# WhatAShot/Electrocardio-Panorama

Measured on AMD Instinct MI355X. Metric: ECG-samples/sec (train step), higher is better.
Workload: dtype f32 (conv products: fp32 operands split into fp16 hi+lo = 22-23 bits, block-scaled, 3 fp16 matrix products each, fp32 accumulate; fp32-class, not IEEE fp32)

## Files before the change

electrocardio_panorama_amd/_lib.py:

```python
import ctypes as C
import os

import torch

_HERE = os.path.dirname(os.path.abspath(__file__))
LIB_PATH = os.path.join(_HERE, "csrc", "libnefnet_hip.so")

NEF_OK = 0
_ERR = {-1: "NEF_E_SHAPE", -2: "NEF_E_NULL", -3: "NEF_E_WORKSPACE", -4: "NEF_E_UNSUPPORTED"}

p = C.c_void_p
i32 = C.c_int
i64 = C.c_int64
f32 = C.c_float
sz = C.c_size_t


class ConvArgs(C.Structure):
    _fields_ = [
        ("x", p), ("wp", p), ("y", p), ("bias", p), ("in_scale", p), ("res", p), ("gate", p), ("mask", p),
        ("x_bs", i64), ("x_gs", i64), ("y_bs", i64), ("y_gs", i64), ("sc_bs", i64), ("sc_gs", i64),
        ("res_bs", i64), ("res_gs", i64), ("gate_bs", i64), ("gate_gs", i64),
        ("B", i32), ("T", i32), ("G", i32), ("Cin_g", i32), ("Cout_g", i32), ("K", i32),
        ("relu", i32), ("gate_scale", f32), ("drop_scale", f32), ("drop_p", f32), ("rng_seed", C.c_uint64),
# ... 92 lines not shown
    "nef_pass_combine_bwd": (i32, [p, p, i32, i32, i32, p]),
    "nef_pass_combine_stats_ws_bytes": (sz, [i32, i32]),
    "nef_pass_combine_fwd_stats": (i32, [p, p, p, p, p, p, p, p, p, p, p, p, sz, i32, i32, i32, f32, f32, p, p]),
    "nef_upsample2_fwd": (i32, [p, p, i64, i32, p]),
    "nef_upsample2_bwd": (i32, [p, p, i64, i32, p]),
    "nef_bn_ws_bytes": (sz, [i32, i32]),
    "nef_bn_train_stats": (i32, [p, p, p, p, p, p, p, p, p, p, sz, i32, i32, i32, i32, f32, f32, p, p]),
    "nef_conv_stats_slots": (i32, [i32, i32]),
    "nef_bn_stats_from_slots": (i32, [p, i32, p, p, p, p, p, p, p, p, p, sz, i32, i32, i32, i32, f32, f32, p, p]),
    "nef_bn_eval_affine": (i32, [p, p, p, p, p, p, i32, f32, p]),
    "nef_fold_bn": (i32, [p, p, p, p, p, p, i32, i32, p]),
    "nef_affine_relu_fwd": (i32, [p, p, p, p, i32, i32, i32, i32, p]),
    "nef_bn_bwd_ws_bytes": (sz, [C.POINTER(BnBwdArgs)]),
    "nef_bn_relu_bwd": (i32, [C.POINTER(BnBwdArgs), p]),
    "nef_bn_bwd_args_bytes": (sz, []),
    "nef_outconv_fwd": (i32, [p, p, p, i32, p, p, p, i32, i32, i32, p]),
    "nef_outconv_bwd_weight": (i32, [p, p, p, p, p, i32, p, p, p, sz, i32, i32, i32, p]),
    "nef_outconv_bwd_data": (i32, [p, p, p, p, i32, i32, i32, p]),
    "nef_outconv_bwd_weight_ws_bytes": (sz, [i32]),
    "nef_loss_ws_bytes": (sz, []),
    "nef_loss_fwd": (i32, [p, p, p, p, p, p, sz, i64, f32, f32, f32, i32, i32, p]),
    "nef_loss_bwd": (i32, [p, p, p, p, p, p, p, p, i64, f32, f32, f32, i32, i32, p]),
    "nef_loss_noise_fwd": (i32, [p, p, p, p, p, p, p, sz, i64, f32, f32, f32, i32, i32, p]),
    "nef_loss_noise_bwd": (i32, [p, p, p, p, p, p, p, p, p, i64, f32, f32, f32, i32, i32, p]),
    "nef_sgd_momentum": (i32, [p, p, p, i64, f32, f32, f32, i32, p, p, p, p]),
    "nef_adam": (i32, [p, p, p, p, i64, f32, C.c_double, C.c_double, f32, f32, f32, p, p, p, p, p]),
    "nef_update": (i32, [C.POINTER(UpdateArgs), p]),
    "nef_update_args_bytes": (sz, []),
    "nef_update_ema": (i32, [C.POINTER(UpdateArgs), C.POINTER(EmaArgs), p]),
    "nef_ema_args_bytes": (sz, []),
# ... 62 lines not shown
```

electrocardio_panorama_amd/csrc/elementwise.hip:

```cpp
#include "nef_common.h"
#include "roi_unpool.h"

namespace {

__global__ void chscale_fwd_kernel(const float* __restrict__ x, const float* __restrict__ s, int64_t s_bs,
                                   float* __restrict__ y, int B, int C, int T) {
    const int64_t rows = (int64_t)B * C;
    const int wave = threadIdx.x >> 6, lane = threadIdx.x & 63;
    for (int64_t row = (int64_t)blockIdx.x * 4 + wave; row < rows; row += (int64_t)gridDim.x * 4) {
        const int b = (int)(row / C), c = (int)(row % C);
        const float f = s[(int64_t)b * s_bs + c];
        const float* xr = x + row * T;
        float* yr = y + row * T;
        for (int t = lane; t < T; t += 64) yr[t] = xr[t] * f;
    }
}

__global__ void chscale_bwd_kernel(const float* __restrict__ gy, const float* __restrict__ x,
                                   const float* __restrict__ s, int64_t s_bs, float* __restrict__ gx,
                                   float* __restrict__ gs, int B, int C, int T, int relu_x) {
    const int64_t rows = (int64_t)B * C;
    const int wave = threadIdx.x >> 6, lane = threadIdx.x & 63;
    for (int64_t row = (int64_t)blockIdx.x * 4 + wave; row < rows; row += (int64_t)gridDim.x * 4) {
        const int b = (int)(row / C), c = (int)(row % C);
// ... 584 lines not shown
        const float af = a[p * C + c], bf = b[p * C + c];
        const float* xr = x + row * L;
        float* yr = y + row * L;
        for (int t = lane; t < L; t += 64) yr[t] = fmaxf(fmaf(xr[t], af, bf), 0.f);
    }
}

__global__ void outconv_go_kernel(const float* __restrict__ gout, const float* __restrict__ out, float* __restrict__ go,
                                  int64_t n) {
    for (int64_t i = (int64_t)blockIdx.x * blockDim.x + threadIdx.x; i < n; i += (int64_t)gridDim.x * blockDim.x) {
        const float o = out[i];
        go[i] = gout[i] * (o * (1.f - o)) / 3.0f;
    }
}

__device__ __forceinline__ nef_f32x4 oc_grad4(const float* __restrict__ gor, int t4, int L, float w0, float w1, float w2) {
    const nef_f32x4 m = *(const nef_f32x4*)(gor + 4 * t4);
    const float lo = t4 > 0 ? gor[4 * t4 - 1] : 0.f;
    const float hi = 4 * t4 + 4 < L ? gor[4 * t4 + 4] : 0.f;
    nef_f32x4 g;
    g[0] = w0 * m[1] + w1 * m[0] + w2 * lo;
    g[1] = w0 * m[2] + w1 * m[1] + w2 * m[0];
    g[2] = w0 * m[3] + w1 * m[2] + w2 * m[1];
    g[3] = w0 * hi + w1 * m[3] + w2 * m[2];
    return g;
}

__device__ __forceinline__ nef_f32x4 up2_adjoint4(const float* __restrict__ gr, int t4, int L) {
    const nef_f32x4 v0 = *(const nef_f32x4*)(gr + 8 * t4), v1 = *(const nef_f32x4*)(gr + 8 * t4 + 4);
    const float lo = t4 > 0 ? gr[8 * t4 - 1] : 0.f;
    const float hi = 8 * t4 + 8 < 2 * L ? gr[8 * t4 + 8] : 0.f;
    nef_f32x4 g;
    g[0] = 0.25f * lo + 0.75f * v0[0] + 0.75f * v0[1] + 0.25f * v0[2];
    g[1] = 0.25f * v0[1] + 0.75f * v0[2] + 0.75f * v0[3] + 0.25f * v1[0];
    g[2] = 0.25f * v0[3] + 0.75f * v1[0] + 0.75f * v1[1] + 0.25f * v1[2];
    g[3] = 0.25f * v1[1] + 0.75f * v1[2] + 0.75f * v1[3] + 0.25f * hi;
    if (t4 == 0) g[0] = up2_bwd_edge(gr, L, 0);
    if (4 * t4 + 3 == L - 1) g[3] = up2_bwd_edge(gr, L, L - 1);
    return g;
}

template <int MODE>
__global__ __launch_bounds__(256) void bn_bwd_partial(const float* __restrict__ gy, const float* __restrict__ x,
                                                      const float* __restrict__ mean, const float* __restrict__ invstd,
                                                      const float* __restrict__ a, const float* __restrict__ b,
                                                      double* __restrict__ part, int P, int Bp, int C, int L,
                                                      const float* __restrict__ ocw) {
    __shared__ double sm[4];
    int bid = blockIdx.x;
    const int sp = bid % BN_SPLIT;
    bid /= BN_SPLIT;
    const int c = bid % C;
    const int p = bid / C;
    const float mf = mean[p * C + c], is = invstd[p * C + c], af = a[p * C + c], bf = b[p * C + c];
    constexpr bool OC = MODE == 1, UPG = MODE == 2;
    const float w0 = OC ? ocw[c * 3] : 0.f, w1 = OC ? ocw[c * 3 + 1] : 0.f, w2 = OC ? ocw[c * 3 + 2] : 0.f;
    double s1 = 0.0, s2 = 0.0;
    if ((L & 3) == 0) {
        const int L4 = L >> 2;
        for (int bb = sp; bb < Bp; bb += BN_SPLIT) {
            const int64_t off = (((int64_t)p * Bp + bb) * C + c) * L;
            const nef_f32x4* xr = (const nef_f32x4*)(x + off);
            const nef_f32x4* gr = (const nef_f32x4*)(gy + off);
            const float* gor = gy + ((int64_t)p * Bp + bb) * L;
            const float* gur = gy + 2 * off;
#pragma unroll 2
            for (int t = threadIdx.x; t < L4; t += 256) {
                const nef_f32x4 xv = xr[t],
                                gv = OC ? oc_grad4(gor, t, L, w0, w1, w2) : (UPG ? up2_adjoint4(gur, t, L) : gr[t]);
#pragma unroll
                for (int e = 0; e < 4; ++e) {
                    const float g = fmaf(xv[e], af, bf) > 0.f ? gv[e] : 0.f;
                    s1 += (double)g;
                    s2 += (double)g * (double)((xv[e] - mf) * is);
                }
            }
        }
    } else {
        for (int bb = sp; bb < Bp; bb += BN_SPLIT) {
            const int64_t off = (((int64_t)p * Bp + bb) * C + c) * L;
            for (int t = threadIdx.x; t < L; t += 256) {
                const float xv = x[off + t];
                const float g = fmaf(xv, af, bf) > 0.f ? gy[off + t] : 0.f;
                s1 += (double)g;
                s2 += (double)g * (double)((xv - mf) * is);
            }
        }
    }
    s1 = nef_block_sum_d(s1, sm);
    s2 = nef_block_sum_d(s2, sm);
    if (threadIdx.x == 0) {
        part[((int64_t)(p * C + c) * BN_SPLIT + sp) * 2] = s1;
        part[((int64_t)(p * C + c) * BN_SPLIT + sp) * 2 + 1] = s2;
    }
}

__global__ void bn_bwd_final(const double* __restrict__ part, float* __restrict__ coef, float* __restrict__ ggamma,
                             float* __restrict__ gbeta, int P, int Bp, int C, int L, int nsplit = BN_SPLIT) {
    const int c = blockIdx.x * blockDim.x + threadIdx.x;
    if (c >= C) return;
    const double n = (double)Bp * (double)L;
    double g1 = 0.0, g2 = 0.0;
    for (int p = 0; p < P; ++p) {
        double s1 = 0.0, s2 = 0.0;
        for (int sp = 0; sp < nsplit; ++sp) {
            s1 += part[((int64_t)(p * C + c) * nsplit + sp) * 2];
            s2 += part[((int64_t)(p * C + c) * nsplit + sp) * 2 + 1];
        }
        coef[(p * C + c) * 2] = (float)(s1 / n);
// ... 136 lines not shown
    double rs[3] = {0.0, 0.0, 0.0};
    for (int t = threadIdx.x; t < L; t += 256) {
        float o[3];
#pragma unroll
        for (int p = 0; p < 3; ++p) {
            const float xv = xr[p][t];
            const float g = fmaf(xv, af[p], bf[p]) > 0.f ? gr[p][t] : 0.f;
            o[p] = af[p] * (g - k1[p] - (xv - mf[p]) * is[p] * k2[p]);
            rs[p] += (double)o[p];
        }
        const int tq = deint ? (t & 1) * (L >> 1) + (t >> 1) : t;
        am[tq] = o[0] + o[2];
        ap[tq] = o[1];
        bm[tq] = o[0] + o[1];
        bp[tq] = o[2];
    }
    if (rowsum) {
#pragma unroll
        for (int p = 0; p < 3; ++p) {
            const double v = nef_block_sum_d(rs[p], sm);
            if (threadIdx.x == 0) rowsum[((int64_t)p * Bp + bb) * C + c] = v;
        }
    }
}

__global__ __launch_bounds__(256) void rowsum_to_channel(const double* __restrict__ rowsum, float* __restrict__ out,
                                                         int NB, int C) {
    __shared__ double sm[4];
    const int c = blockIdx.x;
    double s = 0.0;
// ... 1298 lines not shown
    NEF_REQUIRE(x && a && b && y, NEF_E_NULL);
    NEF_REQUIRE(P > 0 && Bp > 0 && C > 0 && L > 0, NEF_E_SHAPE);
    hipLaunchKernelGGL(affine_relu_fwd_kernel, dim3(nef_stream_grid((int64_t)P * Bp * C, 4)), dim3(256), 0, NEF_ST, x,
                       a, b, y, P, Bp, C, L);
    return nef_launch_status();
}

size_t nef_bn_bwd_args_bytes(void) { return sizeof(nef_bn_bwd_args); }

size_t nef_bn_bwd_ws_bytes(const nef_bn_bwd_args* a) {
    if (!a || a->form < 0 || a->form > 3 || a->P <= 0 || a->Bp <= 0 || a->C <= 0 || a->L <= 0) return 0;
    const size_t go = a->form == 1 ? (size_t)a->P * a->Bp * a->L * sizeof(float) : 0;
    return nef_bn_ws_bytes(a->P, a->C) + (size_t)a->P * a->Bp * a->C * sizeof(double) + go;
}

int nef_bn_relu_bwd(const nef_bn_bwd_args* args, nef_stream_t stream) {
    NEF_ENTER();
    NEF_REQUIRE(args, NEF_E_NULL);
    const nef_bn_bwd_args& a = *args;
    const int P = a.P, Bp = a.Bp, C = a.C, L = a.L, form = a.form, deint = a.phase_major;
    NEF_REQUIRE(a.x && a.mean && a.invstd && a.a && a.b && a.gx && a.ggamma && a.gbeta && a.ws, NEF_E_NULL);
    NEF_REQUIRE(form >= 0 && form <= 3, NEF_E_UNSUPPORTED);
    if (form == 1) {
        NEF_REQUIRE(a.gout && a.out && a.wout, NEF_E_NULL);
        NEF_REQUIRE(!a.g && !a.slots && !deint, NEF_E_UNSUPPORTED);
    } else {
        NEF_REQUIRE(a.g, NEF_E_NULL);
        NEF_REQUIRE(!a.gout && !a.out && !a.wout && !(form == 2 && deint), NEF_E_UNSUPPORTED);
    }
    NEF_REQUIRE(P > 0 && Bp > 0 && C > 0 && L > 0, NEF_E_SHAPE);
    NEF_REQUIRE(form != 3 || P == 3, NEF_E_UNSUPPORTED);
    const int64_t rows = (int64_t)P * Bp * C;
    const bool by_rows = (L & 3) == 0 && rows <= 0x7FFFFFFF;
    switch (form) {
    case 0: NEF_REQUIRE(!deint || by_rows, NEF_E_SHAPE); break;
    case 1: NEF_REQUIRE(by_rows, NEF_E_SHAPE); break;
    case 2: NEF_REQUIRE(by_rows && L >= 8, NEF_E_SHAPE); break;
    case 3: NEF_REQUIRE((int64_t)Bp * C <= 0x7FFFFFFF && (!deint || (L & 1) == 0), NEF_E_SHAPE); break;
    }
    NEF_REQUIRE(!a.slots || (a.nslot > 0 && (int64_t)Bp * a.nslot <= 0x7FFFFFFF), NEF_E_SHAPE);
    NEF_REQUIRE(a.ws_bytes >= nef_bn_bwd_ws_bytes(args), NEF_E_WORKSPACE);
    double* part = (double*)a.ws;
    float* coef = (float*)((char*)a.ws + (size_t)P * C * BN_SPLIT * 2 * sizeof(double));
    double* rowsum = a.gx_chan_sum ? (double*)((char*)a.ws + nef_bn_ws_bytes(P, C)) : nullptr;
    const float* g = a.g;
    if (form == 1) {
        float* go = (float*)((char*)a.ws + nef_bn_ws_bytes(P, C) + (size_t)rows * sizeof(double));
        const int64_t n = (int64_t)P * Bp * L;
        hipLaunchKernelGGL(outconv_go_kernel, dim3(nef_stream_grid(n, 256)), dim3(256), 0, NEF_ST, a.gout, a.out, go, n);
        g = go;
    }
    if (a.slots) {
        hipLaunchKernelGGL(bn_slots_bwd_fused, dim3((unsigned)C), dim3(BNF_THREADS), 0, NEF_ST, a.slots, coef, a.ggamma, a.gbeta, P, Bp, C,
                           L, Bp * a.nslot);
    } else {
        const dim3 grid(P * C * BN_SPLIT);
        if (form == 1)
            hipLaunchKernelGGL(bn_bwd_partial<1>, grid, dim3(256), 0, NEF_ST, g, a.x, a.mean, a.invstd, a.a, a.b, part, P, Bp, C, L,
                               a.wout);
        else if (form == 2)
            hipLaunchKernelGGL(bn_bwd_partial<2>, grid, dim3(256), 0, NEF_ST, g, a.x, a.mean, a.invstd, a.a, a.b, part, P, Bp, C, L,
                               (const float*)nullptr);
        else
            hipLaunchKernelGGL(bn_bwd_partial<0>, grid, dim3(256), 0, NEF_ST, g, a.x, a.mean, a.invstd, a.a, a.b, part, P, Bp, C, L,
                               (const float*)nullptr);
        hipLaunchKernelGGL(bn_bwd_final, dim3((C + 63) / 64), dim3(64), 0, NEF_ST, (const double*)part, coef, a.ggamma, a.gbeta, P, Bp, C,
                           L, BN_SPLIT);
    }
    const dim3 grid((unsigned)rows);
    if (form == 3)
        hipLaunchKernelGGL(bn_bwd_apply_combine3, dim3((unsigned)(Bp * C)), dim3(256), 0, NEF_ST, g, a.x, a.mean, a.invstd, a.a, a.b,
                           (const float*)coef, a.gx, rowsum, Bp, C, L, deint);
    else if (form == 2)
        hipLaunchKernelGGL(bn_bwd_apply_rows<2>, grid, dim3(256), 0, NEF_ST, g, a.x, a.mean, a.invstd, a.a, a.b, (const float*)coef, a.gx,
                           rowsum, Bp, C, L >> 2, (const float*)nullptr);
    else if (form == 1)
        hipLaunchKernelGGL(bn_bwd_apply_rows<1>, grid, dim3(256), 0, NEF_ST, g, a.x, a.mean, a.invstd, a.a, a.b, (const float*)coef, a.gx,
                           rowsum, Bp, C, L >> 2, a.wout);
    else if (by_rows)
        hipLaunchKernelGGL(bn_bwd_apply_rows<0>, grid, dim3(256), 0, NEF_ST, g, a.x, a.mean, a.invstd, a.a, a.b, (const float*)coef, a.gx,
                           rowsum, Bp, C, L >> 2, (const float*)nullptr, deint);
    else
        hipLaunchKernelGGL(bn_bwd_apply, dim3(nef_stream_grid(rows, 4)), dim3(256), 0, NEF_ST, g, a.x, a.mean, a.invstd, a.a, a.b,
                           (const float*)coef, a.gx, rowsum, P, Bp, C, L);
    if (a.gx_chan_sum)
        hipLaunchKernelGGL(rowsum_to_channel, dim3(C), dim3(256), 0, NEF_ST, (const double*)rowsum, a.gx_chan_sum, P * Bp, C);
    return nef_launch_status();
}

int nef_outconv_fwd(const float* x, const float* a, const float* b, int Bp, const float* w, const float* bias,
                    float* out, int N, int C, int L, nef_stream_t stream) {
    NEF_ENTER();
    NEF_REQUIRE(x && w && bias && out, NEF_E_NULL);
    NEF_REQUIRE((a == nullptr) == (b == nullptr), NEF_E_NULL);
    NEF_REQUIRE(N > 0 && C > 0 && C <= OC_MAXC && L > 0 && (!a || Bp > 0), NEF_E_SHAPE);
    if ((L & 3) == 0) {
        const int tiles = (L + 1023) / 1024;
        hipLaunchKernelGGL(outconv_fwd_kernel<true>, dim3((unsigned)((int64_t)N * tiles)), dim3(256), 0, NEF_ST, x, w, bias,
                           out, N, C, L, tiles, a, b, a ? Bp : 1);
        return nef_launch_status();
    }
    const int tiles = (L + 255) / 256;
    hipLaunchKernelGGL(outconv_fwd_kernel<false>, dim3((unsigned)((int64_t)N * tiles)), dim3(256), 0, NEF_ST, x, w, bias,
                       out, N, C, L, tiles, a, b, a ? Bp : 1);
// ... 272 lines not shown
```

electrocardio_panorama_amd/csrc/roi.hip:

```cpp
#include "nef_common.h"
#include "roi_unpool.h"

namespace {

using namespace nef_unpool;

__device__ __forceinline__ float grid_x(const int64_t* __restrict__ roi_b, int j, int s, int T) {
    const float sc = (float)(2.0 / (double)T);
    const float r0 = ((float)roi_b[2 * j] * 0.25f) * sc + (-1.0f);
    const float r1 = ((float)roi_b[2 * j + 1] * 0.25f) * sc + (-1.0f);
    const float step = (r1 - r0) / (float)(BINS - 1);
    return s < BINS / 2 ? r0 + step * (float)s : r1 - step * (float)(BINS - 1 - s);
}

__device__ __forceinline__ float col_weight(float gx) {
    const float ix = ((gx + 1.f) * 1.f - 1.f) * 0.5f;
    const float x0 = floorf(ix);
    const float we = ix - x0;
    const float ww = 1.f - we;
    float w = 0.f;
    if (x0 == 0.f) w += ww;
    if (x0 + 1.f == 0.f) w += we;
    return w;
}
// ... 235 lines not shown
    constexpr int ROW = NSEG * SEGW;
    if (choice_dev) c2 = choice_dev[1];
    const int64_t rows = (int64_t)B * 128;
    const int wave = __builtin_amdgcn_readfirstlane((int)(threadIdx.x >> 6)), lane = threadIdx.x & 63;
    const int s = lane & (SEGW - 1), half = lane >> 5;
    const int64_t per_wave = (rows + (int64_t)gridDim.x * 4 - 1) / ((int64_t)gridDim.x * 4);
    const int64_t row_lo = ((int64_t)blockIdx.x * 4 + wave) * per_wave;
    const int64_t row_hi = row_lo + per_wave < rows ? row_lo + per_wave : rows;
    float* sa = strip_lds + wave * (2 * T + ROW);
    float* sb = sa + T;
    float* pick = sb + T;
    const float fv = (float)V;
    const int64_t pass = (int64_t)B * 256 * T;
    int b_cur = -1;
    SegTable st;
    for (int64_t row = row_lo; row < row_hi; ++row) {
        const int b = (int)(row >> 7), c = (int)(row & 127);
        if (b != b_cur) {
            b_cur = b;
            load_segments(rois + (int64_t)b * NSEG * 2, T, st);
        }
        const float* zr = z2b + (((int64_t)b * V + c2) * 128 + c) * ROW;
#pragma unroll
        for (int u = 0; u < 4; ++u)
            if (u * 64 + lane < ROW) pick[u * 64 + lane] = zr[u * 64 + lane];
        __builtin_amdgcn_fence(__ATOMIC_RELEASE, "wavefront");
        __builtin_amdgcn_wave_barrier();
        const int64_t grow = ((int64_t)b * 256 + 128 + c) * T;
        const float f = q[b * 256 + 128 + c];
        float acc = 0.f;
        constexpr int NU = G == 4 ? 6 : (G == 2 ? 10 : 20);
        const int shift = G == 4 ? (c & 1) * T : 0;
        const int kb = shift / G, ke = (shift + T + G - 1) / G;
        for (int k0 = (kb & ~63) + lane; k0 < ke; k0 += 64 * NU) {
            float ga[NU][G], gb[NU][G], la[NU][G];
// ... 32 lines not shown
                        if (segment_of(st, t, i, sc, jb)) {
                            lerp_src(i, sc, i0, i1, l0, l1);
                            pk = unpool_lerp(l0, pick[jb + i0], l1, pick[jb + i1]);
                        }
                        acc += ga[u][e] * la[u][e] + gb[u][e] * pk;
                        const float gm = f * ga[u][e] / fv;
                        sa[t] = gm + 0.f;
                        sb[t] = gm + f * gb[u][e];
                    }
                }
            }
        }
        __builtin_amdgcn_fence(__ATOMIC_RELEASE, "wavefront");
        __builtin_amdgcn_wave_barrier();
        float ra[(NSEG + 1) / 2] = {0.f, 0.f, 0.f, 0.f}, rb[(NSEG + 1) / 2] = {0.f, 0.f, 0.f, 0.f};
        unpool_gather_row(sa, st, lane, ra);
        unpool_gather_row(sb, st, lane, rb);
        for (int v = 0; v < V; ++v) {
            float* gz = gz2b + (((int64_t)b * V + v) * 128 + c) * ROW;
#pragma unroll
            for (int k = 0; k < (NSEG + 1) / 2; ++k)
                if (2 * k + half < NSEG) gz[(2 * k + half) * SEGW + s] = v == c2 ? rb[k] : ra[k];
        }
        acc = nef_wave_sum(acc);
        if (lane == 0) gq[b * 256 + 128 + c] = acc;
        __builtin_amdgcn_wave_barrier();
    }
}

__global__ void roi_segment_table_kernel(const int64_t* __restrict__ rois, int64_t* __restrict__ seg_start,
                                         int64_t* __restrict__ seg_len, int n) {
    const int i = blockIdx.x * blockDim.x + threadIdx.x;
// ... 101 lines not shown
```

electrocardio_panorama_amd/csrc/roi_unpool.h:

```cpp
#pragma once
#include "nef_common.h"

namespace nef_unpool {

constexpr int NSEG = NEF_N_SEG;
constexpr int BINS = NEF_ROI_BINS;
constexpr int SEGW = 2 * NEF_ROI_BINS;

__device__ __forceinline__ int64_t latent_index(int64_t roi) {
    return (int64_t)((float)roi * 0.25f);
}

struct SegTable { int start[NSEG]; int len[NSEG]; int off[NSEG]; float scale[NSEG]; };

__device__ __forceinline__ bool load_segments(const int64_t* __restrict__ roi_b, int T, SegTable& st) {
    int run = 0;
    bool ok = true;
#pragma unroll
    for (int j = 0; j < NSEG; ++j) {
        const int64_t a = latent_index(roi_b[2 * j]);
        const int64_t e = latent_index(roi_b[2 * j + 1]);
        int64_t len = e - a;
        if (len < 0) { ok = false; len = 0; }
        if (run + len > T) { ok = false; len = T - run; }
// ... 31 lines not shown
    if (s <= 0) return 0;
    int i = (int)ceilf(((float)s + 0.5f) * inv_scale - 0.5f);
    if (i < 0) i = 0;
    if (i > len) i = len;
    if (i > 0 && unpool_left_tap(i - 1, scale) >= s) --i;
    else if (i < len && unpool_left_tap(i, scale) < s) ++i;
    if ((i > 0 && unpool_left_tap(i - 1, scale) >= s) || (i < len && unpool_left_tap(i, scale) < s)) {
#pragma nounroll
        while (i > 0 && unpool_left_tap(i - 1, scale) >= s) --i;
#pragma nounroll
        while (i < len && unpool_left_tap(i, scale) < s) ++i;
    }
    return i;
}

__device__ __forceinline__ void unpool_gather_row(const float* gr, const SegTable& st, int lane, float (&acc_out)[(NSEG + 1) / 2]) {
    const int s = lane & (SEGW - 1), half = lane >> 5;
#pragma unroll
    for (int jj = 0; jj < NSEG + 1; jj += 2) {
        const int j = jj + half;
        if (j >= NSEG) continue;
        const int len = half ? st.len[jj + 1 < NSEG ? jj + 1 : jj] : st.len[jj];
        const int off = half ? st.off[jj + 1 < NSEG ? jj + 1 : jj] : st.off[jj];
        const float sc = half ? st.scale[jj + 1 < NSEG ? jj + 1 : jj] : st.scale[jj];
        float acc = 0.f;
        if (len > 0) {
            const int b0 = unpool_first_reaching(s, len, sc, (float)len * (1.f / SEGW));
            const int nb = __shfl_down(b0, 1), pb = __shfl_up(b0, 1);
            const int b1 = s + 1 < SEGW ? nb : len;
            const int a0 = s > 0 ? pb : b0;
            const float* gp = gr + off;
            float fi = (float)a0 + 0.5f;
            const float sm1 = (float)(s - 1);
            for (int i = a0; i < b0; ++i, fi += 1.f) {
                float src = sc * fi - 0.5f;
                src = src < 0.f ? 0.f : src;
                acc += (src - sm1) * gp[i];
            }
            const float c0 = s == SEGW - 1 ? 1.f : (float)(s + 1), k = s == SEGW - 1 ? 0.f : 1.f;
            for (int i = b0; i < b1; ++i, fi += 1.f) {
                float src = sc * fi - 0.5f;
                src = src < 0.f ? 0.f : src;
                acc += (c0 - k * src) * gp[i];
            }
        }
        acc_out[jj >> 1] = acc;
    }
}

}

NEF_HIDDEN void nef_unpool_mix_fwd_z2(const float* z2b, const int64_t* rois, const float* q, float* latent, float* D2, int32_t* status,
                                      int B, int V, int T, int c2, const int32_t* choice_dev, hipStream_t st);
NEF_HIDDEN void nef_unpool_mix_bwd_z2(const float* gD, const float* latent, const float* z2b, const int64_t* rois, const float* q,
                                      float* gz2b, float* gq, int B, int V, int T, int c2, const int32_t* choice_dev, int group,
                                      hipStream_t st);
```

electrocardio_panorama_amd/engine.py:

```python
import os

import torch
from . import _env

from . import ops
from .ops import GV

N_SEG, ROI_BINS = 7, 16
DROP_P = 0.2
BN_EPS, BN_MOM = 1e-5, 0.1


DROPOUT_SITES = ("W_encoder.layer1.0", "W_encoder.layer1.1", "W_encoder.layer1.2", "w_conv.0", "z1_conv.0",
                 "z2_conv1.0", "z2_conv2.0", "z2_conv2.2")


class DropCfg:

    def __init__(self, training, p=DROP_P, masks=None, seed=0, seed_dev=None):
        self.seed_dev = seed_dev
        self.on = bool(training) and p > 0.0
        self.p = p if self.on else 0.0
        self.scale = 1.0 / (1.0 - p) if self.on else 1.0
        self.masks = masks
# ... 248 lines not shown
            mean = invstd = None
            Bp = N
        if save:
            saved.append((x_in, c, mean, invstd, a, b, pro, up_after, xedge))
        x, pro_in = c, (a, b, Bp)
    out = ops.outconv_fwd(x, P["decoder.4.weight"], P["decoder.4.bias"], pro=pro_in)
    return out, (saved, x, out, passes, pro_in, shared_B)


def decoder_bwd(dsaved, g_out, P, grads, side=None):
    saved, c4, out, passes, pro4 = dsaved[:5]
    shared_B = dsaved[5] if len(dsaved) > 5 else None
    side = side or ops._Inline()
    if len(dsaved) > 5:
        ops.pack_many(_decoder_pack_requests(P, c4.shape[2] // 4, True))
    grads["decoder.4.weight"], grads["decoder.4.bias"] = side.run(
        lambda: ops.outconv_bwd_weight(g_out, out, c4, pro=pro4), g_out, out, c4)
    fuse_last = c4.shape[2] % 4 == 0
    g_is_up = False
    g = None if fuse_last else ops.outconv_bwd_data(g_out, out, P["decoder.4.weight"], c4.shape[1])
    g_slots = None
    poly_first = False
    for li in (3, 2, 1, 0):
        blk, cv, bn, cout = _DEC[li]
        x, c, mean, invstd, a, b, pro, up_after = saved[li][:8]
        xedge = saved[li][8] if len(saved[li]) > 8 else None
        sh0 = li == 0 and shared_B is not None
        Cog_, Cig_ = c.shape[1], x.shape[1] // (2 if sh0 else 1)
        poly_b = bool(up_after and pro[0] & 2 and (not sh0 or pro[0] == 2) and ops.poly_bwd_ok(2 if sh0 else 1, Cog_, Cig_, c.shape[2]))
        pm = bool(poly_b and xedge is not None and ops.poly_w_ok((2 if sh0 else 1) * (shared_B if sh0 else c.shape[0]), 2 if sh0 else 1, Cog_, Cig_, c.shape[2]))
        wname, bname, pre = f"{blk}.double_conv.{cv}.weight", f"{blk}.double_conv.{cv}.bias", f"{blk}.double_conv.{bn}"
        pm0_done = False
        if li == 3 and fuse_last:
            gc, gg, gbeta, gbias = ops.bn_relu_bwd_outconv(g_out, out, P["decoder.4.weight"], c, mean, invstd, a, b, passes)
        elif li == 0 and shared_B is not None and not g_is_up:
            gc, gg, gbeta, gbias = ops.bn_relu_bwd_combine3(g, c, mean, invstd, a, b, slots=g_slots, phase_major=pm)
            pm0_done = pm
        elif g_is_up:
            gc, gg, gbeta, gbias = ops.bn_relu_bwd_up(g, c, mean, invstd, a, b, passes, slots=g_slots)
        else:
            gc, gg, gbeta, gbias = ops.bn_relu_bwd(g, c, P[pre + ".weight"], mean, invstd, a, b, passes,
                                                   with_chan_sum=True, slots=g_slots, phase_major=pm and not sh0)
            pm0_done = pm and not sh0
        grads[pre + ".weight"], grads[pre + ".bias"], grads[bname] = gg, gbeta, gbias
        pm = pm and pm0_done
        if li == 0 and shared_B is not None:
            gp2 = gc if gc.shape[0] == 2 * shared_B else ops.pass_combine_bwd(gc)
            gpv, xv = GV.dense(gp2, 2), GV.dense(x, 2)
            if pm:
# ... 363 lines not shown
```

electrocardio_panorama_amd/ops.py:

```python
import ctypes as C
import contextlib
import itertools
import os
from typing import NamedTuple, Optional

import torch
from . import _env

from . import _lib

N_SEG, ROI_BINS = 7, 16


def _p(t):
    return None if t is None else t.data_ptr()


def _stream():
    return torch.cuda.current_stream().cuda_stream


def _chk(t, dtype=torch.float32):
    assert t.is_cuda and t.dtype == dtype and t.is_contiguous(), (t.device, t.dtype, t.is_contiguous())
    return t
# ... 1249 lines not shown
    wf, bf = torch.empty_like(w), torch.empty_like(bias)
    _lib.check(L.nef_fold_bn(_p(w), _p(bias), _p(a), _p(b), _p(wf), _p(bf), w.shape[0], w.numel() // w.shape[0], _stream()),
               "nef_fold_bn")
    return wf, bf


def affine_relu_fwd(x, a, b, P):
    L = _lib.load()
    _chk(x)
    N, Ct, Ln = x.shape
    y = torch.empty_like(x)
    _lib.check(L.nef_affine_relu_fwd(_p(x), _p(a), _p(b), _p(y), P, N // P, Ct, Ln, _stream()), "nef_affine_relu_fwd")
    return y


def _bn_bwd(form, tag, hbm, x, mean, invstd, a, b, P, gx, chan_sum=True, slots=None, phase_major=False, **grad):
    L = _lib.load()
    N, Ct, Ln = x.shape
    gg = torch.empty(Ct, device=x.device, dtype=torch.float32)
    gb = torch.empty(Ct, device=x.device, dtype=torch.float32)
    gs = torch.empty(Ct, device=x.device, dtype=torch.float32) if chan_sum else None
    A = _lib.BnBwdArgs(x=_p(x), mean=_p(mean), invstd=_p(invstd), a=_p(a), b=_p(b), gx=_p(gx), ggamma=_p(gg), gbeta=_p(gb),
                       gx_chan_sum=_p(gs), slots=_p(slots[0]) if slots else None, nslot=slots[1] if slots else 0, P=P, Bp=N // P,
                       C=Ct, L=Ln, form=form, phase_major=int(phase_major), **{k: _p(t) for k, t in grad.items()})
    A.ws_bytes = L.nef_bn_bwd_ws_bytes(C.byref(A))
    A.ws = _p(workspace(A.ws_bytes, x.device))
    ev = _hbm(tag, *hbm)
    _lib.check(L.nef_bn_relu_bwd(C.byref(A), _stream()), f"nef_bn_relu_bwd form {form}")
    _done(ev)
    return gx, gg, gb, gs


def bn_relu_bwd(gy, x, gamma, mean, invstd, a, b, P, with_chan_sum=False, slots=None, phase_major=False):
    _chk(gy), _chk(x)
    N, Ct, Ln = x.shape
    gx = torch.empty(N, 2 * Ct, Ln // 2, device=x.device, dtype=torch.float32) if phase_major else torch.empty_like(x)
    r = _bn_bwd(0, "bn_relu_bwd", (gy, x, gx), x, mean, invstd, a, b, P, gx, with_chan_sum, slots, phase_major, g=gy)
    return r if with_chan_sum else r[:3]


def bn_relu_bwd_combine3(gy, x, mean, invstd, a, b, slots=None, phase_major=False):
    _chk(gy), _chk(x)
    N, Ct, Ln = x.shape
# ... 4 lines not shown


def bn_relu_bwd_up(gu, x, mean, invstd, a, b, P, slots=None):
    _chk(gu), _chk(x)
    N, Ct, Ln = x.shape
    assert gu.shape == (N, Ct, 2 * Ln)
    gx = torch.empty_like(x)
    return _bn_bwd(2, "bn_relu_bwd_up", (gu, x, gx), x, mean, invstd, a, b, P, gx, slots=slots, g=gu)


def bn_relu_bwd_outconv(gout, out, wout, x, mean, invstd, a, b, P):
    _chk(gout), _chk(out), _chk(x)
    gx = torch.empty_like(x)
    return _bn_bwd(1, "bn_relu_bwd_outconv", (gout, out, x, gout, out, x, gx), x, mean, invstd, a, b, P, gx, gout=gout, out=out,
                   wout=wout)


def outconv_fwd(x, w, bias, pro=None):
    L = _lib.load()
    _chk(x), _chk(w), _chk(bias)
    N, Ct, Ln = x.shape
    out = torch.empty(N, 1, Ln, device=x.device, dtype=torch.float32)
    a, b, Bp = pro if pro is not None else (None, None, 1)
    ev = _hbm("outconv_fwd", x, out)
    _lib.check(L.nef_outconv_fwd(_p(x), _p(a), _p(b), Bp, _p(w), _p(bias), _p(out), N, Ct, Ln, _stream()), "nef_outconv_fwd")
    _done(ev)
    return out


def outconv_bwd_data(gout, out, w, Ct):
# ... 278 lines not shown
```

include/nefnet_hip.h:

```cpp
#ifndef NEFNET_HIP_H
#define NEFNET_HIP_H

#include <stddef.h>
#include <stdint.h>

#ifdef __cplusplus
extern "C" {
#endif

#define NEF_OK 0
#define NEF_E_SHAPE (-1)
#define NEF_E_NULL (-2)
#define NEF_E_WORKSPACE (-3)
#define NEF_E_UNSUPPORTED (-4)

#define NEF_N_SEG 7
#define NEF_ROI_BINS 16

typedef void* nef_stream_t;

int nef_abi_version(void);

int nef_debug_spin_us(float us, int wgs, nef_stream_t stream);

// ... 200 lines not shown
    float* gbeta;
    float* gx_chan_sum;
    const float* slots;
    void* ws;
    size_t ws_bytes;
    int32_t P, Bp, C, L;
    int32_t nslot;
    int32_t form;
    int32_t phase_major;
    int32_t reserved0;
} nef_bn_bwd_args;

int nef_bn_relu_bwd(const nef_bn_bwd_args* a, nef_stream_t stream);
size_t nef_bn_bwd_ws_bytes(const nef_bn_bwd_args* a);
size_t nef_bn_bwd_args_bytes(void);

int nef_outconv_fwd(const float* x, const float* a, const float* b, int Bp, const float* w, const float* bias,
                    float* out, int N, int C, int L, nef_stream_t stream);
int nef_outconv_bwd_weight(const float* gout, const float* out, const float* x, const float* a, const float* b, int Bp,
                           float* gw, float* gb, void* ws, size_t ws_bytes, int N, int C, int L, nef_stream_t stream);
int nef_outconv_bwd_data(const float* gout, const float* out, const float* w, float* gx, int N, int C, int L,
                         nef_stream_t stream);
size_t nef_outconv_bwd_weight_ws_bytes(int C);

size_t nef_loss_ws_bytes(void);
int nef_loss_fwd(const float* pred, const float* pred_p, const float* pred_l, const float* target, float* losses,
                 void* ws, size_t ws_bytes, int64_t n, float f0, float f1, float f2, int reg_l2, int use_mask,
                 nef_stream_t stream);
int nef_loss_bwd(const float* pred, const float* pred_p, const float* pred_l, const float* target,
                 const float* gscale , float* g_pred, float* g_p, float* g_l, int64_t n, float f0,
// ... 95 lines not shown
```

Baseline: 8827.

## Fuse output-conv weight grad into BN backward, add row combine3 and paired unpool gather

The final 1x3 output conv's weight and bias gradients are now accumulated inside the BN/ReLU backward partial-reduction pass, which already reads the activation and output gradient. This drops a separate outconv_bwd_weight pass, which previously could run on a side stream. Separately, a new vectorised, unrolled combine3 apply kernel handles L divisible by 4. The ROI unpool backward now computes gather bounds once per batch and gathers two rows in a single loop. The fusion adds double-precision FMAs and extra block reductions to the BN partial kernel, which may lengthen it.

```diff
diff --git a/electrocardio_panorama_amd/_lib.py b/electrocardio_panorama_amd/_lib.py
--- a/electrocardio_panorama_amd/_lib.py
+++ b/electrocardio_panorama_amd/_lib.py
@@ -130,6 +130,8 @@
     "nef_bn_bwd_ws_bytes": (sz, [C.POINTER(BnBwdArgs)]),
     "nef_bn_relu_bwd": (i32, [C.POINTER(BnBwdArgs), p]),
     "nef_bn_bwd_args_bytes": (sz, []),
+    "nef_bn_relu_bwd_outconv_w": (i32, [C.POINTER(BnBwdArgs), p, p, p]),
+    "nef_bn_relu_bwd_outconv_w_ws_bytes": (sz, [C.POINTER(BnBwdArgs)]),
     "nef_outconv_fwd": (i32, [p, p, p, i32, p, p, p, i32, i32, i32, p]),
     "nef_outconv_bwd_weight": (i32, [p, p, p, p, p, i32, p, p, p, sz, i32, i32, i32, p]),
     "nef_outconv_bwd_data": (i32, [p, p, p, p, i32, i32, i32, p]),
diff --git a/electrocardio_panorama_amd/csrc/elementwise.hip b/electrocardio_panorama_amd/csrc/elementwise.hip
--- a/electrocardio_panorama_amd/csrc/elementwise.hip
+++ b/electrocardio_panorama_amd/csrc/elementwise.hip
@@ -622,16 +622,21 @@
     }
 }
 
-__device__ __forceinline__ nef_f32x4 oc_grad4(const float* __restrict__ gor, int t4, int L, float w0, float w1, float w2) {
+__device__ __forceinline__ nef_f32x4 oc_grad4(const float* __restrict__ gor, int t4, int L, float w0, float w1, float w2, float (&go6)[6]) {
     const nef_f32x4 m = *(const nef_f32x4*)(gor + 4 * t4);
     const float lo = t4 > 0 ? gor[4 * t4 - 1] : 0.f;
     const float hi = 4 * t4 + 4 < L ? gor[4 * t4 + 4] : 0.f;
+    go6[0] = lo, go6[1] = m[0], go6[2] = m[1], go6[3] = m[2], go6[4] = m[3], go6[5] = hi;
     nef_f32x4 g;
     g[0] = w0 * m[1] + w1 * m[0] + w2 * lo;
     g[1] = w0 * m[2] + w1 * m[1] + w2 * m[0];
     g[2] = w0 * m[3] + w1 * m[2] + w2 * m[1];
     g[3] = w0 * hi + w1 * m[3] + w2 * m[2];
     return g;
+}
+__device__ __forceinline__ nef_f32x4 oc_grad4(const float* __restrict__ gor, int t4, int L, float w0, float w1, float w2) {
+    float go6[6];
+    return oc_grad4(gor, t4, L, w0, w1, w2, go6);
 }
 
 __device__ __forceinline__ nef_f32x4 up2_adjoint4(const float* __restrict__ gr, int t4, int L) {
@@ -648,12 +653,13 @@
     return g;
 }
 
-template <int MODE>
+template <int MODE, bool OCW = false>
 __global__ __launch_bounds__(256) void bn_bwd_partial(const float* __restrict__ gy, const float* __restrict__ x,
                                                       const float* __restrict__ mean, const float* __restrict__ invstd,
                                                       const float* __restrict__ a, const float* __restrict__ b,
                                                       double* __restrict__ part, int P, int Bp, int C, int L,
-                                                      const float* __restrict__ ocw) {
+                                                      const float* __restrict__ ocw, double* __restrict__ wpart = nullptr) {
+    static_assert(!OCW || MODE == 1, "the last conv's weight gradient rides on the pass that rebuilds its input gradient");
     __shared__ double sm[4];
     int bid = blockIdx.x;
     const int sp = bid % BN_SPLIT;
@@ -664,6 +670,7 @@
     constexpr bool OC = MODE == 1, UPG = MODE == 2;
     const float w0 = OC ? ocw[c * 3] : 0.f, w1 = OC ? ocw[c * 3 + 1] : 0.f, w2 = OC ? ocw[c * 3 + 2] : 0.f;
     double s1 = 0.0, s2 = 0.0;
+    double gw0 = 0.0, gw1 = 0.0, gw2 = 0.0, gsum = 0.0;
     if ((L & 3) == 0) {
         const int L4 = L >> 2;
         for (int bb = sp; bb < Bp; bb += BN_SPLIT) {
@@ -674,14 +681,23 @@
             const float* gur = gy + 2 * off;
 #pragma unroll 2
             for (int t = threadIdx.x; t < L4; t += 256) {
+                float go6[6];
                 const nef_f32x4 xv = xr[t],
-                                gv = OC ? oc_grad4(gor, t, L, w0, w1, w2) : (UPG ? up2_adjoint4(gur, t, L) : gr[t]);
+                                gv = OC ? oc_grad4(gor, t, L, w0, w1, w2, go6) : (UPG ? up2_adjoint4(gur, t, L) : gr[t]);
 #pragma unroll
                 for (int e = 0; e < 4; ++e) {
                     const float g = fmaf(xv[e], af, bf) > 0.f ? gv[e] : 0.f;
                     s1 += (double)g;
                     s2 += (double)g * (double)((xv[e] - mf) * is);
+                    if constexpr (OCW) {
+                        const double act = (double)fmaxf(fmaf(xv[e], af, bf), 0.f);
+                        gw0 = fma((double)go6[e + 2], act, gw0);
+                        gw1 = fma((double)go6[e + 1], act, gw1);
+                        gw2 = fma((double)go6[e], act, gw2);
+                    }
                 }
+                if constexpr (OCW)
+                    if (c == 0) gsum += (((double)go6[1] + (double)go6[2]) + (double)go6[3]) + (double)go6[4];
             }
         }
     } else {
@@ -701,6 +717,31 @@
         part[((int64_t)(p * C + c) * BN_SPLIT + sp) * 2] = s1;
         part[((int64_t)(p * C + c) * BN_SPLIT + sp) * 2 + 1] = s2;
     }
+    if constexpr (OCW) {
+        gw0 = nef_block_sum_d(gw0, sm);
+        gw1 = nef_block_sum_d(gw1, sm);
+        gw2 = nef_block_sum_d(gw2, sm);
+        gsum = nef_block_sum_d(gsum, sm);
+        if (threadIdx.x == 0) {
+            double* w = wpart + ((int64_t)(p * C + c) * BN_SPLIT + sp) * 4;
+            w[0] = gw0, w[1] = gw1, w[2] = gw2, w[3] = gsum;
+        }
+    }
+}
+
+__global__ void bn_bwd_outconv_w_final(const double* __restrict__ wpart, float* __restrict__ gw, float* __restrict__ gb, int P,
+                                       int C) {
+    const int i = blockIdx.x * blockDim.x + threadIdx.x;
+    if (i > C * 3) return;
+    const int c = i < C * 3 ? i / 3 : 0, k = i < C * 3 ? i % 3 : 3;
+    double tot = 0.0;
+    for (int p = 0; p < P; ++p) {
+        double sp_sum = 0.0;
+        for (int sp = 0; sp < BN_SPLIT; ++sp) sp_sum += wpart[((int64_t)(p * C + c) * BN_SPLIT + sp) * 4 + k];
+        tot += sp_sum;
+    }
+    if (i < C * 3) gw[i] = (float)tot;
+    else gb[0] = (float)tot;
 }
 
 __global__ void bn_bwd_final(const double* __restrict__ part, float* __restrict__ coef, float* __restrict__ ggamma,
@@ -867,6 +908,76 @@
         ap[tq] = o[1];
         bm[tq] = o[0] + o[1];
         bp[tq] = o[2];
+    }
+    if (rowsum) {
+#pragma unroll
+        for (int p = 0; p < 3; ++p) {
+            const double v = nef_block_sum_d(rs[p], sm);
+            if (threadIdx.x == 0) rowsum[((int64_t)p * Bp + bb) * C + c] = v;
+        }
+    }
+}
+
+__global__ __launch_bounds__(256) void bn_bwd_apply_combine3_rows(const float* __restrict__ gy, const float* __restrict__ x,
+                                                                  const float* __restrict__ mean,
+                                                                  const float* __restrict__ invstd, const float* __restrict__ a,
+                                                                  const float* __restrict__ b, const float* __restrict__ coef,
+                                                                  float* __restrict__ gP2, double* __restrict__ rowsum, int Bp,
+                                                                  int C, int L4, int deint) {
+    __shared__ double sm[4];
+    constexpr int U = 2;
+    const int bb = blockIdx.x / C, c = blockIdx.x % C;
+    const int L = 4 * L4;
+    float mf[3], is[3], af[3], bf[3], k1[3], k2[3];
+    const nef_f32x4* xr[3];
+    const nef_f32x4* gr[3];
+#pragma unroll
+    for (int p = 0; p < 3; ++p) {
+        const int pc = p * C + c;
+        mf[p] = mean[pc]; is[p] = invstd[pc]; af[p] = a[pc]; bf[p] = b[pc];
+        k1[p] = coef[pc * 2]; k2[p] = coef[pc * 2 + 1];
+        const int64_t off = (((int64_t)p * Bp + bb) * C + c) * L;
+        xr[p] = (const nef_f32x4*)(x + off);
+        gr[p] = (const nef_f32x4*)(gy + off);
+    }
+    float* const dst[4] = {gP2 + ((int64_t)bb * 2 * C + c) * L, gP2 + ((int64_t)(Bp + bb) * 2 * C + c) * L,
+                           gP2 + ((int64_t)bb * 2 * C + C + c) * L, gP2 + ((int64_t)(Bp + bb) * 2 * C + C + c) * L};
+    double rs[3] = {0.0, 0.0, 0.0};
+    for (int t0 = 0; t0 < L4; t0 += 256 * U) {
+        nef_f32x4 xv[U][3], gv[U][3];
+#pragma unroll
+        for (int u = 0; u < U; ++u) {
+            const int t = t0 + u * 256 + threadIdx.x;
+            if (t < L4) {
+#pragma unroll
+                for (int p = 0; p < 3; ++p) xv[u][p] = xr[p][t], gv[u][p] = gr[p][t];
+            }
+        }
+#pragma unroll
+        for (int u = 0; u < U; ++u) {
+            const int t = t0 + u * 256 + threadIdx.x;
+            if (t < L4) {
+                nef_f32x4 o[3];
+#pragma unroll
+                for (int p = 0; p < 3; ++p)
+#pragma unroll
+                    for (int e = 0; e < 4; ++e) {
+                        const float xe = xv[u][p][e];
+                        const float g = fmaf(xe, af[p], bf[p]) > 0.f ? gv[u][p][e] : 0.f;
+                        o[p][e] = af[p] * (g - k1[p] - (xe - mf[p]) * is[p] * k2[p]);
+                        rs[p] += (double)o[p][e];
+                    }
+                const nef_f32x4 v[4] = {o[0] + o[2], o[1], o[0] + o[1], o[2]};
+#pragma unroll
+                for (int r = 0; r < 4; ++r) {
+                    if (deint) {
+                        ((nef_f32x2*)dst[r])[t] = nef_f32x2{v[r][0], v[r][2]};
+                        ((nef_f32x2*)(dst[r] + 2 * L4))[t] = nef_f32x2{v[r][1], v[r][3]};
+                    } else
+                        ((nef_f32x4*)dst[r])[t] = v[r];
+                }
+            }
+        }
     }
     if (rowsum) {
 #pragma unroll
@@ -2195,9 +2306,14 @@
     return nef_bn_ws_bytes(a->P, a->C) + (size_t)a->P * a->Bp * a->C * sizeof(double) + go;
 }
 
-int nef_bn_relu_bwd(const nef_bn_bwd_args* args, nef_stream_t stream) {
-    NEF_ENTER();
-    NEF_REQUIRE(args, NEF_E_NULL);
+static size_t bn_bwd_wpart_offset(const nef_bn_bwd_args* a) { return (nef_bn_bwd_ws_bytes(a) + 7) & ~(size_t)7; }
+
+size_t nef_bn_relu_bwd_outconv_w_ws_bytes(const nef_bn_bwd_args* a) {
+    if (!a || a->form != 1 || a->P <= 0 || a->Bp <= 0 || a->C <= 0 || a->L <= 0) return 0;
+    return bn_bwd_wpart_offset(a) + (size_t)a->P * a->C * BN_SPLIT * 4 * sizeof(double);
+}
+
+static int bn_relu_bwd_launch(const nef_bn_bwd_args* args, float* gw, float* gb, nef_stream_t stream) {
     const nef_bn_bwd_args& a = *args;
     const int P = a.P, Bp = a.Bp, C = a.C, L = a.L, form = a.form, deint = a.phase_major;
     NEF_REQUIRE(a.x && a.mean && a.invstd && a.a && a.b && a.gx && a.ggamma && a.gbeta && a.ws, NEF_E_NULL);
@@ -2220,7 +2336,7 @@
     case 3: NEF_REQUIRE((int64_t)Bp * C <= 0x7FFFFFFF && (!deint || (L & 1) == 0), NEF_E_SHAPE); break;
     }
     NEF_REQUIRE(!a.slots || (a.nslot > 0 && (int64_t)Bp * a.nslot <= 0x7FFFFFFF), NEF_E_SHAPE);
-    NEF_REQUIRE(a.ws_bytes >= nef_bn_bwd_ws_bytes(args), NEF_E_WORKSPACE);
+    NEF_REQUIRE(a.ws_bytes >= (gw ? nef_bn_relu_bwd_outconv_w_ws_bytes(args) : nef_bn_bwd_ws_bytes(args)), NEF_E_WORKSPACE);
     double* part = (double*)a.ws;
     float* coef = (float*)((char*)a.ws + (size_t)P * C * BN_SPLIT * 2 * sizeof(double));
     double* rowsum = a.gx_chan_sum ? (double*)((char*)a.ws + nef_bn_ws_bytes(P, C)) : nullptr;
@@ -2236,7 +2352,13 @@
                            L, Bp * a.nslot);
     } else {
         const dim3 grid(P * C * BN_SPLIT);
-        if (form == 1)
+        if (gw) {
+            double* wpart = (double*)((char*)a.ws + bn_bwd_wpart_offset(args));
+            hipLaunchKernelGGL((bn_bwd_partial<1, true>), grid, dim3(256), 0, NEF_ST, g, a.x, a.mean, a.invstd, a.a, a.b, part, P, Bp, C,
+                               L, a.wout, wpart);
+            hipLaunchKernelGGL(bn_bwd_outconv_w_final, dim3((C * 3 + 1 + 63) / 64), dim3(64), 0, NEF_ST, (const double*)wpart, gw, gb,
+                               P, C);
+        } else if (form == 1)
             hipLaunchKernelGGL(bn_bwd_partial<1>, grid, dim3(256), 0, NEF_ST, g, a.x, a.mean, a.invstd, a.a, a.b, part, P, Bp, C, L,
                                a.wout);
         else if (form == 2)
@@ -2249,7 +2371,10 @@
                            L, BN_SPLIT);
     }
     const dim3 grid((unsigned)rows);
-    if (form == 3)
+    if (form == 3 && (L & 3) == 0)
+        hipLaunchKernelGGL(bn_bwd_apply_combine3_rows, dim3((unsigned)(Bp * C)), dim3(256), 0, NEF_ST, g, a.x, a.mean, a.invstd, a.a,
+                           a.b, (const float*)coef, a.gx, rowsum, Bp, C, L >> 2, deint);
+    else if (form == 3)
         hipLaunchKernelGGL(bn_bwd_apply_combine3, dim3((unsigned)(Bp * C)), dim3(256), 0, NEF_ST, g, a.x, a.mean, a.invstd, a.a, a.b,
                            (const float*)coef, a.gx, rowsum, Bp, C, L, deint);
     else if (form == 2)
@@ -2269,6 +2394,20 @@
     return nef_launch_status();
 }
 
+int nef_bn_relu_bwd(const nef_bn_bwd_args* args, nef_stream_t stream) {
+    NEF_ENTER();
+    NEF_REQUIRE(args, NEF_E_NULL);
+    return bn_relu_bwd_launch(args, nullptr, nullptr, stream);
+}
+
+int nef_bn_relu_bwd_outconv_w(const nef_bn_bwd_args* args, float* gw, float* gb, nef_stream_t stream) {
+    NEF_ENTER();
+    NEF_REQUIRE(args, NEF_E_NULL);
+    NEF_REQUIRE(args->form == 1, NEF_E_UNSUPPORTED);
+    NEF_REQUIRE(gw && gb, NEF_E_NULL);
+    return bn_relu_bwd_launch(args, gw, gb, stream);
+}
+
 int nef_outconv_fwd(const float* x, const float* a, const float* b, int Bp, const float* w, const float* bias,
                     float* out, int N, int C, int L, nef_stream_t stream) {
     NEF_ENTER();
diff --git a/electrocardio_panorama_amd/csrc/roi.hip b/electrocardio_panorama_amd/csrc/roi.hip
--- a/electrocardio_panorama_amd/csrc/roi.hip
+++ b/electrocardio_panorama_amd/csrc/roi.hip
@@ -273,11 +273,13 @@
     const int64_t pass = (int64_t)B * 256 * T;
     int b_cur = -1;
     SegTable st;
+    GatherBounds bnd;
     for (int64_t row = row_lo; row < row_hi; ++row) {
         const int b = (int)(row >> 7), c = (int)(row & 127);
         if (b != b_cur) {
             b_cur = b;
             load_segments(rois + (int64_t)b * NSEG * 2, T, st);
+            unpool_gather_bounds(st, lane, bnd);
         }
         const float* zr = z2b + (((int64_t)b * V + c2) * 128 + c) * ROW;
 #pragma unroll
@@ -340,8 +342,7 @@
         __builtin_amdgcn_fence(__ATOMIC_RELEASE, "wavefront");
         __builtin_amdgcn_wave_barrier();
         float ra[(NSEG + 1) / 2] = {0.f, 0.f, 0.f, 0.f}, rb[(NSEG + 1) / 2] = {0.f, 0.f, 0.f, 0.f};
-        unpool_gather_row(sa, st, lane, ra);
-        unpool_gather_row(sb, st, lane, rb);
+        unpool_gather_row2(sa, sb, st, bnd, lane, ra, rb);
         for (int v = 0; v < V; ++v) {
             float* gz = gz2b + (((int64_t)b * V + v) * 128 + c) * ROW;
 #pragma unroll
diff --git a/electrocardio_panorama_amd/csrc/roi_unpool.h b/electrocardio_panorama_amd/csrc/roi_unpool.h
--- a/electrocardio_panorama_amd/csrc/roi_unpool.h
+++ b/electrocardio_panorama_amd/csrc/roi_unpool.h
@@ -69,37 +69,90 @@
     return i;
 }
 
+__device__ __forceinline__ int unpool_gather_len(const SegTable& st, int jj, int half) {
+    return half ? (jj + 1 < NSEG ? st.len[jj + 1 < NSEG ? jj + 1 : jj] : 0) : st.len[jj];
+}
+__device__ __forceinline__ int unpool_gather_b0(const SegTable& st, int jj, int s, int half) {
+    const int len = unpool_gather_len(st, jj, half);
+    const float sc = half ? st.scale[jj + 1 < NSEG ? jj + 1 : jj] : st.scale[jj];
+    return len > 0 ? unpool_first_reaching(s, len, sc, (float)len * (1.f / SEGW)) : 0;
+}
+__device__ __forceinline__ void unpool_gather_ends(const SegTable& st, int jj, int s, int half, int b0, int& a0, int& b1) {
+    const int nb = __shfl_down(b0, 1), pb = __shfl_up(b0, 1);
+    b1 = s + 1 < SEGW ? nb : unpool_gather_len(st, jj, half);
+    a0 = s > 0 ? pb : b0;
+}
+
 __device__ __forceinline__ void unpool_gather_row(const float* gr, const SegTable& st, int lane, float (&acc_out)[(NSEG + 1) / 2]) {
     const int s = lane & (SEGW - 1), half = lane >> 5;
 #pragma unroll
     for (int jj = 0; jj < NSEG + 1; jj += 2) {
         const int j = jj + half;
         if (j >= NSEG) continue;
-        const int len = half ? st.len[jj + 1 < NSEG ? jj + 1 : jj] : st.len[jj];
         const int off = half ? st.off[jj + 1 < NSEG ? jj + 1 : jj] : st.off[jj];
         const float sc = half ? st.scale[jj + 1 < NSEG ? jj + 1 : jj] : st.scale[jj];
+        const int b0 = unpool_gather_b0(st, jj, s, half);
+        int a0, b1;
+        unpool_gather_ends(st, jj, s, half, b0, a0, b1);
         float acc = 0.f;
-        if (len > 0) {
-            const int b0 = unpool_first_reaching(s, len, sc, (float)len * (1.f / SEGW));
-            const int nb = __shfl_down(b0, 1), pb = __shfl_up(b0, 1);
-            const int b1 = s + 1 < SEGW ? nb : len;
-            const int a0 = s > 0 ? pb : b0;
-            const float* gp = gr + off;
-            float fi = (float)a0 + 0.5f;
-            const float sm1 = (float)(s - 1);
-            for (int i = a0; i < b0; ++i, fi += 1.f) {
-                float src = sc * fi - 0.5f;
-                src = src < 0.f ? 0.f : src;
-                acc += (src - sm1) * gp[i];
-            }
-            const float c0 = s == SEGW - 1 ? 1.f : (float)(s + 1), k = s == SEGW - 1 ? 0.f : 1.f;
-            for (int i = b0; i < b1; ++i, fi += 1.f) {
-                float src = sc * fi - 0.5f;
-                src = src < 0.f ? 0.f : src;
-                acc += (c0 - k * src) * gp[i];
-            }
+        const float* gp = gr + off;
+        float fi = (float)a0 + 0.5f;
+        const float sm1 = (float)(s - 1);
+        for (int i = a0; i < b0; ++i, fi += 1.f) {
+            float src = sc * fi - 0.5f;
+            src = src < 0.f ? 0.f : src;
+            acc += (src - sm1) * gp[i];
+        }
+        const float c0 = s == SEGW - 1 ? 1.f : (float)(s + 1), k = s == SEGW - 1 ? 0.f : 1.f;
+        for (int i = b0; i < b1; ++i, fi += 1.f) {
+            float src = sc * fi - 0.5f;
+            src = src < 0.f ? 0.f : src;
+            acc += (c0 - k * src) * gp[i];
         }
         acc_out[jj >> 1] = acc;
+    }
+}
+
+struct GatherBounds { int b0[(NSEG + 1) / 2]; };
+
+__device__ __forceinline__ void unpool_gather_bounds(const SegTable& st, int lane, GatherBounds& bnd) {
+    const int s = lane & (SEGW - 1), half = lane >> 5;
+#pragma unroll
+    for (int jj = 0; jj < NSEG + 1; jj += 2) bnd.b0[jj >> 1] = unpool_gather_b0(st, jj, s, half);
+}
+
+__device__ __forceinline__ void unpool_gather_row2(const float* ga, const float* gb, const SegTable& st, const GatherBounds& bnd,
+                                                   int lane, float (&acc_a)[(NSEG + 1) / 2], float (&acc_b)[(NSEG + 1) / 2]) {
+    const int s = lane & (SEGW - 1), half = lane >> 5;
+    const float sm1 = (float)(s - 1);
+    const float c0 = s == SEGW - 1 ? 1.f : (float)(s + 1), k = s == SEGW - 1 ? 0.f : 1.f;
+#pragma unroll
+    for (int jj = 0; jj < NSEG + 1; jj += 2) {
+        const int off = half ? st.off[jj + 1 < NSEG ? jj + 1 : jj] : st.off[jj];
+        const float sc = half ? st.scale[jj + 1 < NSEG ? jj + 1 : jj] : st.scale[jj];
+        const int b0 = bnd.b0[jj >> 1];
+        int a0, b1;
+        unpool_gather_ends(st, jj, s, half, b0, a0, b1);
+        const float* pa = ga + off;
+        const float* pb = gb + off;
+        float xa = 0.f, xb = 0.f;
+        float fi = (float)a0 + 0.5f;
+        for (int i = a0; i < b0; ++i, fi += 1.f) {
+            float src = sc * fi - 0.5f;
+            src = src < 0.f ? 0.f : src;
+            const float w = src - sm1;
+            xa += w * pa[i];
+            xb += w * pb[i];
+        }
+        for (int i = b0; i < b1; ++i, fi += 1.f) {
+            float src = sc * fi - 0.5f;
+            src = src < 0.f ? 0.f : src;
+            const float w = c0 - k * src;
+            xa += w * pa[i];
+            xb += w * pb[i];
+        }
+        acc_a[jj >> 1] = xa;
+        acc_b[jj >> 1] = xb;
     }
 }
 
diff --git a/electrocardio_panorama_amd/engine.py b/electrocardio_panorama_amd/engine.py
--- a/electrocardio_panorama_amd/engine.py
+++ b/electrocardio_panorama_amd/engine.py
@@ -286,9 +286,10 @@
     side = side or ops._Inline()
     if len(dsaved) > 5:
         ops.pack_many(_decoder_pack_requests(P, c4.shape[2] // 4, True))
-    grads["decoder.4.weight"], grads["decoder.4.bias"] = side.run(
-        lambda: ops.outconv_bwd_weight(g_out, out, c4, pro=pro4), g_out, out, c4)
     fuse_last = c4.shape[2] % 4 == 0
+    if not fuse_last:
+        grads["decoder.4.weight"], grads["decoder.4.bias"] = side.run(
+            lambda: ops.outconv_bwd_weight(g_out, out, c4, pro=pro4), g_out, out, c4)
     g_is_up = False
     g = None if fuse_last else ops.outconv_bwd_data(g_out, out, P["decoder.4.weight"], c4.shape[1])
     g_slots = None
@@ -304,7 +305,8 @@
         wname, bname, pre = f"{blk}.double_conv.{cv}.weight", f"{blk}.double_conv.{cv}.bias", f"{blk}.double_conv.{bn}"
         pm0_done = False
         if li == 3 and fuse_last:
-            gc, gg, gbeta, gbias = ops.bn_relu_bwd_outconv(g_out, out, P["decoder.4.weight"], c, mean, invstd, a, b, passes)
+            gc, gg, gbeta, gbias, grads["decoder.4.weight"], grads["decoder.4.bias"] = ops.bn_relu_bwd_outconv_w(
+                g_out, out, P["decoder.4.weight"], c, mean, invstd, a, b, passes)
         elif li == 0 and shared_B is not None and not g_is_up:
             gc, gg, gbeta, gbias = ops.bn_relu_bwd_combine3(g, c, mean, invstd, a, b, slots=g_slots, phase_major=pm)
             pm0_done = pm
diff --git a/electrocardio_panorama_amd/ops.py b/electrocardio_panorama_amd/ops.py
--- a/electrocardio_panorama_amd/ops.py
+++ b/electrocardio_panorama_amd/ops.py
@@ -1287,7 +1287,7 @@
     return y
 
 
-def _bn_bwd(form, tag, hbm, x, mean, invstd, a, b, P, gx, chan_sum=True, slots=None, phase_major=False, **grad):
+def _bn_bwd(form, tag, hbm, x, mean, invstd, a, b, P, gx, chan_sum=True, slots=None, phase_major=False, outconv_w=None, **grad):
     L = _lib.load()
     N, Ct, Ln = x.shape
     gg = torch.empty(Ct, device=x.device, dtype=torch.float32)
@@ -1296,10 +1296,13 @@
     A = _lib.BnBwdArgs(x=_p(x), mean=_p(mean), invstd=_p(invstd), a=_p(a), b=_p(b), gx=_p(gx), ggamma=_p(gg), gbeta=_p(gb),
                        gx_chan_sum=_p(gs), slots=_p(slots[0]) if slots else None, nslot=slots[1] if slots else 0, P=P, Bp=N // P,
                        C=Ct, L=Ln, form=form, phase_major=int(phase_major), **{k: _p(t) for k, t in grad.items()})
-    A.ws_bytes = L.nef_bn_bwd_ws_bytes(C.byref(A))
+    A.ws_bytes = (L.nef_bn_relu_bwd_outconv_w_ws_bytes if outconv_w else L.nef_bn_bwd_ws_bytes)(C.byref(A))
     A.ws = _p(workspace(A.ws_bytes, x.device))
     ev = _hbm(tag, *hbm)
-    _lib.check(L.nef_bn_relu_bwd(C.byref(A), _stream()), f"nef_bn_relu_bwd form {form}")
+    if outconv_w:
+        _lib.check(L.nef_bn_relu_bwd_outconv_w(C.byref(A), _p(outconv_w[0]), _p(outconv_w[1]), _stream()), "nef_bn_relu_bwd_outconv_w")
+    else:
+        _lib.check(L.nef_bn_relu_bwd(C.byref(A), _stream()), f"nef_bn_relu_bwd form {form}")
     _done(ev)
     return gx, gg, gb, gs
 
@@ -1334,6 +1337,16 @@
     gx = torch.empty_like(x)
     return _bn_bwd(1, "bn_relu_bwd_outconv", (gout, out, x, gout, out, x, gx), x, mean, invstd, a, b, P, gx, gout=gout, out=out,
                    wout=wout)
+
+
+def bn_relu_bwd_outconv_w(gout, out, wout, x, mean, invstd, a, b, P):
+    _chk(gout), _chk(out), _chk(x)
+    gx = torch.empty_like(x)
+    gw = torch.empty(1, x.shape[1], 3, device=x.device, dtype=torch.float32)
+    gb = torch.empty(1, device=x.device, dtype=torch.float32)
+    r = _bn_bwd(1, "bn_relu_bwd_outconv_w", (gout, out, x, gout, out, x, gx), x, mean, invstd, a, b, P, gx, outconv_w=(gw, gb),
+                gout=gout, out=out, wout=wout)
+    return (*r, gw, gb)
 
 
 def outconv_fwd(x, w, bias, pro=None):
diff --git a/include/nefnet_hip.h b/include/nefnet_hip.h
--- a/include/nefnet_hip.h
+++ b/include/nefnet_hip.h
@@ -238,6 +238,8 @@
 int nef_bn_relu_bwd(const nef_bn_bwd_args* a, nef_stream_t stream);
 size_t nef_bn_bwd_ws_bytes(const nef_bn_bwd_args* a);
 size_t nef_bn_bwd_args_bytes(void);
+int nef_bn_relu_bwd_outconv_w(const nef_bn_bwd_args* a, float* gw, float* gb, nef_stream_t stream);
+size_t nef_bn_relu_bwd_outconv_w_ws_bytes(const nef_bn_bwd_args* a);
 
 int nef_outconv_fwd(const float* x, const float* a, const float* b, int Bp, const float* w, const float* bias,
                     float* out, int N, int C, int L, nef_stream_t stream);
```

After: 8901, median of 6. Within noise of the previous version (+0.8%).
